# NilanEkanayake/TiTok-Video

Hardware: AMD Instinct MI355X
Metric: video clips/sec encode+decode (whole node) (higher is better)
Workload: dtype bf16

## Files before the change

include/titok_hip.h:

```cpp
#ifndef TITOK_HIP_H
#define TITOK_HIP_H

#include <stdint.h>

#ifdef __cplusplus
extern "C" {
#endif

#define TTV_OK 0
#define TTV_ERR_INVALID 1
#define TTV_ERR_LAUNCH 2
#define TTV_ERR_UNSUPPORTED 3

#define TTV_BF16 0
#define TTV_F32 1

#define TTV_ENCODER 0
#define TTV_DECODER 1

#define TTV_MAX_FSQ 8
#define TTV_MAX_TOKEN 64
#define TTV_MAX_CLIPS_PER_LAUNCH 64

const char* ttv_error_string(void);
// ... 324 lines not shown
  const void* pool_proj_w; const void* pool_proj_b;
  const float* pool_norm2_w; const float* pool_norm2_b;
  const void* pool_fc1_w; const void* pool_fc1_b;
  const void* pool_fc2_w; const void* pool_fc2_b;
} ttv_vjepa_weights;

int ttv_jedi_preprocess(void* const* clips, const int32_t* dims, int n_clips, int dtype, void* out, void* stream);
int64_t ttv_vjepa_workspace_bytes(int n);
int ttv_vjepa_features(const ttv_vjepa_weights* w, const void* x, int n, float* feats, int finetuned, void* workspace,
                       int64_t workspace_bytes, void* stream);

#define TTV_VJEPA_EPI_STORE 0
#define TTV_VJEPA_EPI_GELU 1
#define TTV_VJEPA_EPI_RESID 2
int ttv_vjepa_layernorm(const float* x, int ldx, int rows, int width, const float* w1, const float* b1, float eps1, const float* w2,
                        const float* b2, float eps2, float* y32, int ld32, void* y16, int ld16, void* stream);
int ttv_vjepa_linear(const void* x, int ldx, const void* w, int ldw, const void* bias, int M, int N, int K, int epilogue,
                     const float* resid, int ldr, int resid_rows, void* y, int ldy, void* stream);
int ttv_vjepa_pool_attention(const void* q, const void* kv, int n, int rows, void* out, void* stream);

#define TTV_KC_ATTENTION 1
#define TTV_KC_GEMM_QKV 2
#define TTV_KC_GEMM_GEGLU 3
#define TTV_KC_GEMM_RESID 4
#define TTV_KC_GEMM_STORE 5
#define TTV_KC_RMSNORM 6
#define TTV_KC_PATCH 7
#define TTV_KC_ROWS 8
int ttv_prof_begin(int kernel_class, int max_records);
enum {
  TTV_DBG_NO_STORES = 1,
  TTV_DBG_K256_NO_PANEL_DMA = 2,
  TTV_DBG_MLP_NO_WEIGHT_DMA = 2,
  TTV_DBG_K256_NO_TILE_RELOAD = 4,
  TTV_DBG_MLP_NO_GEGLU = 4,
  TTV_DBG_K256_NO_EPILOGUE_MATH = 8,
  TTV_DBG_MLP_TILES8 = 8,
  TTV_DBG_MLP_NO_P2 = 16,
  TTV_DBG_MLP_PAIRS_ONLY = 32,
  TTV_DBG_MLP_TILES4 = 64,
  TTV_DBG_GEMM_TILE160 = 128,
  TTV_DBG_GEMM_TILE128 = 256,
  TTV_DBG_GEMM_T256 = 512,
  TTV_DBG_MLP_TILES9 = 512,
  TTV_DBG_GEMM_NO_T256 = 1024,
  TTV_DBG_MX_UNFUSED_QUANT = 2048,
  TTV_DBG_SPLIT3_NO_IMAGES = 4096,
  TTV_DBG_SPLIT3_NO_DMA = 8192,
  TTV_DBG_K256_GENERAL = 16384,
  TTV_DBG_QKV256_OFF = 32768,
  TTV_DBG_QKV256_WS = 131072,
  TTV_DBG_ENC_ALL_ROWS = 524288,
  TTV_DBG_ATTN_NO_SWP = 1048576,
  TTV_DBG_DEC_ALL_BLOCKS = 2097152
};
int ttv_debug_set(int flags);
int ttv_debug_stamps(void* device_buffer);
int ttv_prof_end(double* total_ms, int* count);

#ifdef __cplusplus
}
#endif
#endif
```

titok_video_amd/_lib.py:

```python
from __future__ import annotations

import ctypes as C
import os
import threading

import torch

from . import switches

TTV_BF16, TTV_F32 = 0, 1
TTV_ENCODER, TTV_DECODER = 0, 1
TTV_MAX_FSQ = 8
TTV_MAX_TOKEN = 64
TTV_MAX_CLIPS_PER_LAUNCH = 64

DBG_NO_STORES = 1
DBG_K256_NO_PANEL_DMA = 2
DBG_MLP_NO_WEIGHT_DMA = 2
DBG_K256_NO_TILE_RELOAD = 4
DBG_MLP_NO_GEGLU = 4
DBG_K256_NO_EPILOGUE_MATH = 8
DBG_MLP_TILES8 = 8
DBG_MLP_NO_P2 = 16
DBG_MLP_PAIRS_ONLY = 32
DBG_MLP_TILES4 = 64
DBG_GEMM_TILE160 = 128
DBG_GEMM_TILE128 = 256
DBG_GEMM_T256 = 512
DBG_MLP_TILES9 = 512
DBG_GEMM_NO_T256 = 1024
DBG_MX_UNFUSED_QUANT = 2048
DBG_SPLIT3_NO_IMAGES = 4096
DBG_SPLIT3_NO_DMA = 8192
DBG_K256_GENERAL = 16384
DBG_QKV256_OFF = 32768
DBG_QKV256_WS = 131072
DBG_ENC_ALL_ROWS = 524288
DBG_ATTN_NO_SWP = 1048576
DBG_DEC_ALL_BLOCKS = 2097152

_HERE = os.path.dirname(os.path.abspath(__file__))
LIB_PATH = switches.text("TTV_LIB_PATH") or os.path.join(_HERE, "libtitok_hip.so")

i32, i64, f32, vp = C.c_int32, C.c_int64, C.c_float, C.c_void_p


class FsqParams(C.Structure):
    _fields_ = [("n", i32), ("levels", i32 * TTV_MAX_FSQ), ("basis", i32 * TTV_MAX_FSQ),
                ("half_l", f32 * TTV_MAX_FSQ), ("offset", f32 * TTV_MAX_FSQ), ("shift", f32 * TTV_MAX_FSQ),
                ("half_width", f32 * TTV_MAX_FSQ)]


class TowerDims(C.Structure):
    _fields_ = [("kind", i32), ("dtype", i32), ("width", i32), ("layers", i32), ("q_heads", i32), ("kv_heads", i32),
                ("head_dim", i32), ("inner", i32), ("patch_t", i32), ("patch_h", i32), ("patch_w", i32),
                ("pix_channels", i32), ("token_size", i32), ("eps", f32), ("alpha", f32)]


class NextQkv(C.Structure):
    _fields_ = [("qkv", vp), ("ld", i32), ("rope_cs", vp), ("rows", i32), ("rope_q_end", i32), ("rope_k_begin", i32), ("rope_k_end", i32)]


class LayerWeights(C.Structure):
    _fields_ = [("pre_ln", vp), ("to_qkv", vp), ("out_proj", vp), ("ffd_norm", vp), ("w12", vp), ("w3", vp),
                ("attn_post_ln", vp), ("ffd_post_ln", vp), ("to_qkv_pn", vp), ("w12_pn", vp), ("mlp_pack", vp), ("mlp_pack_qkv_rows", i32), ("qkv_q_prescaled", i32),
                ("to_qkv_qs", vp), ("to_qkv_f8", vp), ("to_qkv_f8_scale", vp), ("w12_f8", vp), ("w12_f8_scale", vp),
                ("to_qkv_mx", vp), ("w12_mx", vp), ("out_proj_f8", vp), ("out_proj_f8_scale", vp), ("out_proj_mx", vp),
                ("w3_f8", vp), ("w3_f8_scale", vp), ("w3_mx", vp)]


class TowerWeights(C.Structure):
    _fields_ = [("proj_in_w", vp), ("proj_in_b", vp), ("mask_token", vp), ("ln_pre_t", vp), ("ln_pre_p", vp),
                ("ln_post", vp), ("proj_out_w", vp), ("proj_out_b", vp), ("layers", C.POINTER(LayerWeights)), ("proj_out_pn", vp),
                ("f32_split3", i32)]


class Batch(C.Structure):
    _fields_ = [("n_clips", i32), ("total_rows", i32), ("sum_tokens", i32), ("sum_patches", i32),
                ("max_patches_per_clip", i32), ("n_qblocks", i32), ("cu_seqlens", vp), ("latent_rows", vp),
                ("patch_rows", vp), ("clip_desc", vp), ("qblocks", vp), ("rope_cs", vp), ("blocks64", vp), ("row_seq", vp),
                ("n_blocks64", i32), ("qblocks_paired", i32), ("qblocks_all_full", i32), ("items64", vp), ("n_items64", i32),
                ("rope_ids", vp), ("rope_base", vp), ("qblocks_latent", vp), ("n_qblocks_latent", i32), ("qblocks_patch", vp),
                ("n_qblocks_patch", i32)]


class LayerWeightsT(C.Structure):
    _fields_ = [("to_qkv_t", vp), ("out_proj_t", vp), ("w12_t", vp), ("w3_t", vp)]


class TowerWeightsT(C.Structure):
    _fields_ = [("proj_in_t", vp), ("proj_out_t", vp), ("layers", C.POINTER(LayerWeightsT))]

# ... 200 lines not shown
```

titok_video_amd/csrc/ttv_api.hip:

```cpp
#include <stdarg.h>
#include <stdio.h>
#include <stdlib.h>
#include <string.h>

#include "ttv_common.h"
#include "ttv_kernels.h"

static thread_local char g_err[512] = "";

void ttv_set_error(const char* fmt, ...) {
  va_list ap;
  va_start(ap, fmt);
  vsnprintf(g_err, sizeof(g_err), fmt, ap);
  va_end(ap);
}

int g_ttv_prof_class = 0;
bool ttv_sw_enc_latent_last() { static const bool v = ttv_env_flag("TTV_ENC_LATENT_LAST", true); return v; }
bool ttv_sw_keel_f32sum() { static const bool v = ttv_env_flag("TTV_KEEL_F32SUM", false); return v; }
bool ttv_sw_fused_patch() { static const bool v = ttv_env_flag("TTV_FUSED_PATCH", true); return v; }
bool ttv_sw_attn_pipe() { static const bool v = ttv_env_flag("TTV_ATTN_PIPE", false); return v; }
float ttv_sw_attn_thr() { static const float v = ttv_env_float("TTV_ATTN_THR", 8.0f); return v; }
thread_local int g_ttv_debug = 0;
long long* g_ttv_stamps = nullptr;
static hipEvent_t* g_prof_start = nullptr;
static hipEvent_t* g_prof_stop = nullptr;
static int g_prof_cap = 0, g_prof_n = 0;

TtvProfScope::TtvProfScope(int cls, hipStream_t stream) : slot(-1), s(stream) {
  if (g_ttv_prof_class != 0 && cls == g_ttv_prof_class && g_prof_n < g_prof_cap) {
    slot = g_prof_n++;
    (void)hipEventRecord(g_prof_start[slot], s);
  }
}
TtvProfScope::~TtvProfScope() {
  if (slot >= 0) (void)hipEventRecord(g_prof_stop[slot], s);
}

#define TTV_TRY(expr)            \
  do {                           \
    int rc__ = (expr);           \
    if (rc__ != TTV_OK) return rc__; \
  } while (0)

static inline int esize(int dtype) { return dtype == TTV_BF16 ? 2 : 4; }
static inline int64_t align_up(int64_t v) { return (v + 255) & ~(int64_t)255; }

struct TowerWs {
  char *x, *xn, *qkv, *ao, *h, *pa, *pb;
  char *xl, *aol;
  char *f8, *f8mx;
  float* y32;
  float* rstd;
  int64_t total;
};

static TowerWs carve(const ttv_tower_dims* d, const ttv_batch* b, char* base) {
  const int64_t e = esize(d->dtype);
  const int64_t L = b->total_rows, P = b->sum_patches;
  const int64_t g = (int64_t)d->kv_heads * d->head_dim;
  const int64_t pd = (int64_t)d->pix_channels * d->patch_t * d->patch_h * d->patch_w;
  int64_t off = 0;
  TowerWs w;
  auto take = [&](int64_t bytes) { char* p = base ? base + off : nullptr; off += align_up(bytes); return p; };
  w.x = take(L * d->width * e);
  w.xn = take(L * d->width * e);
  w.qkv = take(L * (2 * d->width + 2 * g) * e);
  w.ao = take(L * d->width * e);
  w.y32 = (float*)take(L * d->width * 4);
  w.h = take(L * d->inner * e);
  w.pa = take(P * pd * e);
  w.pb = take(P * d->width * e);
  w.rstd = (float*)take(L * 4);
// ... 454 lines not shown
  TTV_CHECK_ARG(dtype == TTV_BF16 && head_dim == 64, "attention64: bf16, head_dim 64 only");
  return ttvk_attention64(qkvg, ld, out, ldo, cu_seqlens, items, n_items, q_heads, kv_heads, flags, (hipStream_t)stream);
}

int ttv_patch_gather(const void* const* clips, const int32_t* clip_desc, int clip0, int n_clips, int patch_t, int patch_h, int patch_w,
                     int channels, void* patches, int ld, int dtype, int max_patches_per_clip, void* stream) {
  TTV_CHECK_ARG(n_clips == 0 || (clips && clip_desc && patches), "patch_gather: null buffer");
  return ttvk_patch_copy(false, (void* const*)clips, clip_desc, clip0, n_clips, patch_t, patch_h, patch_w, channels, patches, ld, dtype, max_patches_per_clip, (hipStream_t)stream);
}

int ttv_patch_scatter(const void* patches, int ld, const int32_t* clip_desc, int clip0, int n_clips, int patch_t, int patch_h, int patch_w,
                      int channels, void* const* clips, int dtype, int max_patches_per_clip, void* stream) {
  TTV_CHECK_ARG(n_clips == 0 || (clips && clip_desc && patches), "patch_scatter: null buffer");
  return ttvk_patch_copy(true, clips, clip_desc, clip0, n_clips, patch_t, patch_h, patch_w, channels, (void*)patches, ld, dtype, max_patches_per_clip, (hipStream_t)stream);
}

int64_t ttv_tower_workspace_bytes(const ttv_tower_dims* dims, const ttv_batch* batch) {
  if (check_dims(dims, batch) != TTV_OK) return -1;
  return carve(dims, batch, nullptr).total;
}

int ttv_encoder_forward(const ttv_tower_dims* d, const ttv_tower_weights* w, const ttv_batch* b, const void* const* clips,
                        const ttv_fsq_params* fsq, float* z, void* codes, int32_t* indices, float* bounded, void* workspace,
                        int64_t workspace_bytes, void* stream) {
  TTV_TRY(check_dims(d, b));
  TTV_CHECK_ARG(d->kind == TTV_ENCODER, "encoder_forward: dims.kind is not TTV_ENCODER");
  TTV_CHECK_ARG(w && w->layers && clips && workspace, "encoder_forward: null argument");
  TTV_CHECK_ARG(fsq || z, "encoder_forward: neither fsq nor z requested");
  TTV_CHECK_ARG(!fsq || (codes && indices), "encoder_forward: fsq needs codes and indices buffers");
  hipStream_t s = (hipStream_t)stream;
  TowerWs ws = carve(d, b, (char*)workspace);
  TTV_CHECK_ARG(ws.total <= workspace_bytes, "encoder_forward: workspace too small (%lld < %lld)", (long long)workspace_bytes, (long long)ws.total);
  const int dm = d->width, dt = d->dtype, P = b->sum_patches;
  const int pd = d->pix_channels * d->patch_t * d->patch_h * d->patch_w;

  static const bool use_fused_patch = ttv_sw_fused_patch();
  auto pow2 = [](int v) { return v > 0 && (v & (v - 1)) == 0; };
  const bool gather = use_fused_patch && dt == TTV_BF16 && d->patch_w == 8 && pow2(d->patch_t) && pow2(d->patch_h) &&
                      b->n_clips <= TTV_MAX_CLIPS_PER_LAUNCH && b->row_seq && pd % 64 == 0 && pd != 256;
  if (!gather) {
    for (int c0 = 0; c0 < b->n_clips; c0 += TTV_MAX_CLIPS_PER_LAUNCH) {
      const int n = b->n_clips - c0 < TTV_MAX_CLIPS_PER_LAUNCH ? b->n_clips - c0 : TTV_MAX_CLIPS_PER_LAUNCH;
      TTV_TRY(ttvk_patch_copy(false, (void* const*)(clips + c0), b->clip_desc, c0, n, d->patch_t, d->patch_h, d->patch_w, d->pix_channels, ws.pa, pd, dt, b->max_patches_per_clip, s));
    }
  }
  GemmArgs a = {};
  a.dtype = dt; a.x = ws.pa; a.ldx = pd; a.w = w->proj_in_w; a.ldw = pd; a.M = P; a.N = dm; a.K = pd; a.y = ws.pb; a.ldy = dm;
  a.bias = w->proj_in_b; a.add_scalar = w->mask_token;
  a.split3 = (dt == TTV_F32 && w->f32_split3) ? 1 : 0;
  if (gather) {
    a.gather = 1; a.clips = (void* const*)clips; a.n_clips = b->n_clips; a.clip_desc = b->clip_desc; a.patch_rows = b->patch_rows;
    a.row_seq = b->row_seq; a.patch_t = d->patch_t; a.patch_h = d->patch_h; a.patch_w = d->patch_w;
  }
  TTV_TRY(ttvk_gemm(EPI_STORE, a, s));
  TTV_TRY(ttvk_rmsnorm(ws.pb, dt, dm, nullptr, ws.x, dt, dm, b->patch_rows, w->ln_pre_p, P, dm, d->eps, s));
  TTV_TRY(ttvk_fill_const_rows(ws.x, dt, dm, b->latent_rows, b->sum_tokens, dm, w->mask_token, w->ln_pre_t, d->eps, s));

  TTV_TRY(run_layers(d, w, b, ws, s));

  TTV_TRY(ttvk_enc_tail(ws.x, dt, dm, b->latent_rows, b->sum_tokens, dm, w->ln_post, d->eps, w->proj_out_w, w->proj_out_b, d->token_size, fsq, z, codes, indices, bounded, s));
  return TTV_OK;
}

int ttv_decoder_forward(const ttv_tower_dims* d, const ttv_tower_weights* w, const ttv_batch* b, const void* codes,
                        void* const* clips_out, void* workspace, int64_t workspace_bytes, void* stream) {
  TTV_TRY(check_dims(d, b));
  TTV_CHECK_ARG(d->kind == TTV_DECODER, "decoder_forward: dims.kind is not TTV_DECODER");
  TTV_CHECK_ARG(w && w->layers && codes && clips_out && workspace, "decoder_forward: null argument");
  hipStream_t s = (hipStream_t)stream;
  TowerWs ws = carve(d, b, (char*)workspace);
  TTV_CHECK_ARG(ws.total <= workspace_bytes, "decoder_forward: workspace too small (%lld < %lld)", (long long)workspace_bytes, (long long)ws.total);
  const int dm = d->width, dt = d->dtype, P = b->sum_patches;
  const int pd = d->pix_channels * d->patch_t * d->patch_h * d->patch_w;

  TTV_TRY(ttvk_dec_embed(codes, d->token_size, w->proj_in_w, w->proj_in_b, w->mask_token, w->ln_pre_t, ws.x, dt, dm, b->latent_rows, b->sum_tokens, dm, d->eps, s));
  TTV_TRY(ttvk_fill_const_rows(ws.x, dt, dm, b->patch_rows, P, dm, w->mask_token, w->ln_pre_p, d->eps, s));

  TTV_TRY(run_layers(d, w, b, ws, s));

  GemmArgs a = {};
  a.dtype = dt; a.w = w->proj_out_w; a.ldw = dm; a.M = P; a.N = pd; a.K = dm; a.y = ws.pa; a.ldy = pd; a.ldx = dm;
  a.split3 = (dt == TTV_F32 && w->f32_split3) ? 1 : 0;
  a.bias = w->proj_out_b;
  if (dt == TTV_BF16 && dm == 256 && w->proj_out_pn && pd % 8 == 0) {
    a.x = ws.x; a.x_rows = b->patch_rows; a.w = w->proj_out_pn; a.prenorm = 1; a.eps = d->eps;
  } else {
    TTV_TRY(ttvk_rmsnorm(ws.x, dt, dm, b->patch_rows, ws.pb, dt, dm, nullptr, w->ln_post, P, dm, d->eps, s));
    a.x = ws.pb;
  }
  static const bool use_fused_patch = ttv_sw_fused_patch();
  auto pow2 = [](int v) { return v > 0 && (v & (v - 1)) == 0; };
  if (use_fused_patch && dt == TTV_BF16 && dm == 256 && d->patch_w == 8 && pow2(d->patch_t) && pow2(d->patch_h) &&
      b->n_clips <= TTV_MAX_CLIPS_PER_LAUNCH && b->row_seq && pd % 64 == 0) {
    a.clips = clips_out; a.n_clips = b->n_clips; a.clip_desc = b->clip_desc; a.patch_rows = b->patch_rows; a.row_seq = b->row_seq;
    a.patch_t = d->patch_t; a.patch_h = d->patch_h; a.patch_w = d->patch_w;
    return ttvk_gemm(EPI_STORE_PATCH, a, s);
  }
  TTV_TRY(ttvk_gemm(EPI_STORE, a, s));
  for (int c0 = 0; c0 < b->n_clips; c0 += TTV_MAX_CLIPS_PER_LAUNCH) {
    const int n = b->n_clips - c0 < TTV_MAX_CLIPS_PER_LAUNCH ? b->n_clips - c0 : TTV_MAX_CLIPS_PER_LAUNCH;
    TTV_TRY(ttvk_patch_copy(true, clips_out + c0, b->clip_desc, c0, n, d->patch_t, d->patch_h, d->patch_w, d->pix_channels, ws.pa, pd, dt, b->max_patches_per_clip, s));
  }
  return TTV_OK;
}

int ttv_rope_table_build(const float* base_cos, const float* base_sin, int n_ids, int n_freqs, const int32_t* clip_desc, const int32_t* cu_seqlens,
                         const int32_t* row_seq, float* rope_cs, int total_rows, void* stream) {
  TTV_CHECK_ARG(total_rows == 0 || (base_cos && base_sin && clip_desc && cu_seqlens && row_seq && rope_cs), "rope_table_build: null buffer");
  TTV_CHECK_ARG(n_freqs >= 1 && 3 * n_freqs <= 32 && n_ids >= 1, "rope_table_build: bad table shape");
// ... 183 lines not shown
```

titok_video_amd/csrc/ttv_common.h:

```cpp
#pragma once
#include <hip/hip_runtime.h>
#include <stdint.h>
#include <stdlib.h>

#include "../../include/titok_hip.h"

typedef __bf16 bf16_t;
typedef __attribute__((ext_vector_type(8))) __bf16 bf16x8;
typedef __attribute__((ext_vector_type(4))) __bf16 bf16x4;
typedef __attribute__((ext_vector_type(2))) __bf16 bf16x2;
typedef __attribute__((ext_vector_type(4))) float f32x4;
typedef __attribute__((ext_vector_type(16))) float f32x16;

#define TTV_WAVE 64

void ttv_set_error(const char* fmt, ...);
#define TTV_CHECK_ARG(cond, ...)          \
  do {                                    \
    if (!(cond)) {                        \
      ttv_set_error(__VA_ARGS__);         \
      return TTV_ERR_INVALID;             \
    }                                     \
  } while (0)
#define TTV_CHECK_LAUNCH(what)                                            \
// ... 100 lines not shown
  const unsigned b0 = b[0], b1 = b[1];
  return __uint_as_float(b0) + __uint_as_float(b1);
}
__device__ __forceinline__ float quad16_max(float v) {
  const unsigned u = __float_as_uint(v);
  const auto a = __builtin_amdgcn_permlane16_swap(u, u, false, false);
  const unsigned a0 = a[0], a1 = a[1];
  const float s = fmaxf(__uint_as_float(a0), __uint_as_float(a1));
  const unsigned t = __float_as_uint(s);
  const auto b = __builtin_amdgcn_permlane32_swap(t, t, false, false);
  const unsigned b0 = b[0], b1 = b[1];
  return fmaxf(__uint_as_float(b0), __uint_as_float(b1));
}
__device__ __forceinline__ float pair32_sum(float v) {
  const unsigned u = __float_as_uint(v);
  const auto b = __builtin_amdgcn_permlane32_swap(u, u, false, false);
  const unsigned b0 = b[0], b1 = b[1];
  return __uint_as_float(b0) + __uint_as_float(b1);
}
__device__ __forceinline__ uint4 xchg16_pair(uint2 p0, uint2 p1) {
  const auto x = __builtin_amdgcn_permlane16_swap(p0.x, p1.x, false, false);
  const auto y = __builtin_amdgcn_permlane16_swap(p0.y, p1.y, false, false);
  const unsigned x0 = x[0], x1 = x[1], y0 = y[0], y1 = y[1];
  return make_uint4(x0, y0, x1, y1);
}

extern int g_ttv_prof_class;
extern thread_local int g_ttv_debug;
extern long long* g_ttv_stamps;
struct TtvProfScope {
  int slot;
  hipStream_t s;
  TtvProfScope(int cls, hipStream_t stream);
  ~TtvProfScope();
};

static inline int ttv_cdiv(int a, int b) { return (a + b - 1) / b; }

static inline bool ttv_env_flag(const char* name, bool default_on) {
  const char* v = getenv(name);
  return default_on ? !(v && v[0] == '0') : (v && v[0] == '1');
}
static inline int ttv_env_int(const char* name, int dflt) {
  const char* v = getenv(name);
  return v ? atoi(v) : dflt;
}
static inline float ttv_env_float(const char* name, float dflt) {
  const char* v = getenv(name);
  return v ? (float)atof(v) : dflt;
}
bool ttv_sw_enc_latent_last();
bool ttv_sw_keel_f32sum();
bool ttv_sw_fused_patch();
bool ttv_sw_attn_pipe();
float ttv_sw_attn_thr();

__device__ __forceinline__ float ttv_cubic_src(int dst, float scale) { return fmaf(scale, (float)dst + 0.5f, -0.5f); }
__device__ __forceinline__ int ttv_cubic_floor(int dst, float scale) { return (int)floorf(ttv_cubic_src(dst, scale)); }
__device__ __forceinline__ void cubic_taps(int dst, int n_in, int n_out, int (&idx)[4], float (&w)[4]) {
  const float scale = (float)n_in / (float)n_out;
  const float src = ttv_cubic_src(dst, scale);
  const float fl = floorf(src);
  const float t = src - fl;
  const int i0 = (int)fl;
  constexpr float A = -0.75f;
  auto c1 = [](float x) { return ((A + 2.f) * x - (A + 3.f)) * x * x + 1.f; };
  auto c2 = [](float x) { return ((A * x - 5.f * A) * x + 8.f * A) * x - 4.f * A; };
  w[0] = c2(t + 1.f); w[1] = c1(t); w[2] = c1(1.f - t); w[3] = c2(2.f - t);
#pragma unroll
  for (int k = 0; k < 4; ++k) {
    const int j = i0 - 1 + k;
    idx[k] = j < 0 ? 0 : (j > n_in - 1 ? n_in - 1 : j);
  }
}
typedef float f32x2 __attribute__((ext_vector_type(2)));
__device__ __forceinline__ float geglu_fast(float g, float x) {
  const float gc = __builtin_amdgcn_fmed3f(g, -8.0f, 8.0f);
  const float g2 = gc * gc;
  float q = fmaf(g2, 1.014262858e-03f, -1.067757308e-01f);
  q = fmaf(q, g2, -2.301121361e+00f);
  const float e = __builtin_amdgcn_exp2f(q * gc);
  return (g * __builtin_amdgcn_rcpf(1.0f + e)) * x;
}
__device__ __forceinline__ f32x2 geglu_pair_fast(f32x2 g, f32x2 x) { return (f32x2){geglu_fast(g.x, x.x), geglu_fast(g.y, x.y)}; }

__device__ __forceinline__ void geglu_fast8(const float (&g)[8], const float (&x)[8], float (&h)[8]) {
  float a[8], e[8];
#pragma unroll
  for (int k = 0; k < 8; ++k) {
    const float gc = __builtin_amdgcn_fmed3f(g[k], -8.0f, 8.0f);
    const float g2 = gc * gc;
    float q = fmaf(g2, 1.014262858e-03f, -1.067757308e-01f);
    q = fmaf(q, g2, -2.301121361e+00f);
    a[k] = q * gc;
  }
  __builtin_amdgcn_sched_barrier(0);
#pragma unroll
  for (int k = 0; k < 8; ++k) e[k] = __builtin_amdgcn_exp2f(a[k]);
  __builtin_amdgcn_sched_barrier(0);
#pragma unroll
  for (int k = 0; k < 8; ++k) e[k] = 1.0f + e[k];
  __builtin_amdgcn_sched_barrier(0);
#pragma unroll
  for (int k = 0; k < 8; ++k) e[k] = __builtin_amdgcn_rcpf(e[k]);
  __builtin_amdgcn_sched_barrier(0);
#pragma unroll
// ... 3 lines not shown
```

titok_video_amd/csrc/ttv_gemm.hip:

```cpp
#include <stdlib.h>

#include "ttv_common.h"
#include "ttv_kernels.h"

struct GemmDev {
  const void* x; const void* w; void* y;
  const void* bias; const float* add_scalar; const void* resid; const float* rope_cs;
  int ldx, ldw, ldy, ldr;
  int M, N, K;
  int w_rows;
  float alpha;
  int rope_q_end, rope_k_begin, rope_k_end;
  float eps;
  int debug;
  const float* norm_gain;
  ClipPtrs clips;
  const int* clip_desc; const int* patch_rows; const int* row_seq;
  const int* x_rows;
  const float* row_scale;
  const int* rope_ids; const float* rope_base;
  const float* x_scale; const float* w_scale;
  float* sum_f32; int ld_sum;
  void* y2; int ldy2; const float* norm_gain2;
  int split3;
// ... 1175 lines not shown
    }
    __builtin_amdgcn_s_waitcnt(0x0F70);
    __syncthreads();
    if (it + 1 < it1) {
      LOADA(af[0], buf ^ 1, 0);
      if (K256_DEPTH == 3) LOADA(af[1], buf ^ 1, 1);
    }

    int tok[2];
#pragma unroll
    for (int j = 0; j < 2; ++j) {
      tok[j] = tile * K256_TT + wave * 32 + j * 16 + l15;
      if (PRENORM && !(p.debug & TTV_DBG_K256_NO_EPILOGUE_MATH)) {
#pragma unroll
        for (int i = 0; i < 4; ++i) acc[i][j] *= rstd[j];
      }
    }
    if (DUAL) {
      int feat[2] = {panel * FO + kq * 4, panel * FO + 16 + kq * 4};
      f32x4 ax[2][2] = {{acc[0][0], acc[0][1]}, {acc[1][0], acc[1][1]}};
      f32x4 ag[2][2] = {{acc[2][0], acc[2][1]}, {acc[3][0], acc[3][1]}};
      epilogue_tile<EPI, bf16_t, 2, 2>(p, tok, feat, ax, ag, kq);
    } else if (EPI == EPI_QKV_ROPE) {
      int feat[4];
#pragma unroll
      for (int i = 0; i < 4; ++i) feat[i] = panel * FO + i * 16 + kq * 4;
      const int f_first = panel * FO;
      if (!(p.debug & TTV_DBG_K256_NO_EPILOGUE_MATH) && (f_first < p.rope_q_end || (f_first >= p.rope_k_begin && f_first < p.rope_k_end))) {
#pragma unroll
        for (int i = 0; i < 4; ++i)
#pragma unroll
          for (int j = 0; j < 2; ++j) {
            const f32x4 a = acc[i][j];
            acc[i][j] = (f32x4){a[0] * rc[i][j].x - a[1] * rs[i][j].x, a[0] * rs[i][j].x + a[1] * rc[i][j].x,
                                a[2] * rc[i][j].y - a[3] * rs[i][j].y, a[2] * rs[i][j].y + a[3] * rc[i][j].y};
          }
      }
      epilogue_tile<EPI_STORE, bf16_t, 4, 2>(p, tok, feat, acc, acc, kq);
    } else {
      int feat[4];
#pragma unroll
      for (int i = 0; i < 4; ++i) feat[i] = panel * FO + i * 16 + kq * 4;
      epilogue_tile<EPI, bf16_t, 4, 2>(p, tok, feat, acc, acc, kq, EPI == EPI_STORE_PATCH ? pdst : nullptr);
    }
  }
#undef WROWIDX
#undef GLDS_PANEL
#undef LOADA
#undef MFMA8
}

#include "ttv_qkv256.inc"
#include "ttv_qkv256ws.inc"

#define ROW_TT 64

__global__ __launch_bounds__(256, 2) void k_gemm_k256_rownorm(GemmDev p, int n_tiles) {
  __shared__ uint4 wl[2][K256_ROWS * 32];
  const int tid = threadIdx.x, lane = tid & 63, wave = tid >> 6;
  const int l15 = lane & 15, kq = lane >> 4;
  if ((int)blockIdx.x >= n_tiles) return;
  const bf16_t* W = (const bf16_t*)p.w;
  const bf16_t* X = (const bf16_t*)p.x;
  const int srow = tid >> 5, sch = tid & 31;
  uint4 st0, st1, st2, st3, st4, st5, st6, st7;
#define WROWN(panel_, i_) (*reinterpret_cast<const uint4*>(W + (size_t)((panel_) * 64 + srow + 8 * (i_)) * p.ldw + sch * 8))
#define GLOADN(panel_)                                                                                       \
  do {                                                                                                       \
    st0 = WROWN(panel_, 0); st1 = WROWN(panel_, 1); st2 = WROWN(panel_, 2); st3 = WROWN(panel_, 3);          \
    st4 = WROWN(panel_, 4); st5 = WROWN(panel_, 5); st6 = WROWN(panel_, 6); st7 = WROWN(panel_, 7);          \
  } while (0)
#define LIDXN(i_) ((srow + 8 * (i_)) * 32 + ((sch & 16) | ((sch & 15) ^ ((srow + 8 * (i_)) & 15))))
#define LSTOREN(buf_)                                                                                        \
  do {                                                                                                       \
    wl[buf_][LIDXN(0)] = st0; wl[buf_][LIDXN(1)] = st1; wl[buf_][LIDXN(2)] = st2; wl[buf_][LIDXN(3)] = st3;  \
    wl[buf_][LIDXN(4)] = st4; wl[buf_][LIDXN(5)] = st5; wl[buf_][LIDXN(6)] = st6; wl[buf_][LIDXN(7)] = st7;  \
  } while (0)

  GLOADN(0);
  LSTOREN(0);
  __syncthreads();
  for (int tile = blockIdx.x; tile < n_tiles; tile += gridDim.x) {
    const bool last_tile = tile + (int)gridDim.x >= n_tiles;
    int t = tile * ROW_TT + wave * 16 + l15;
    const bool tvalid = t < p.M;
    t = tvalid ? t : p.M - 1;
    bf16x8 bfr[8];
    {
      const bf16_t* xr = X + (size_t)t * p.ldx + kq * 8;
#pragma unroll
      for (int s8 = 0; s8 < 8; ++s8) bfr[s8] = *reinterpret_cast<const bf16x8*>(xr + s8 * 32);
    }
    f32x4 acc[16];
#pragma unroll
    for (int i = 0; i < 16; ++i) acc[i] = (f32x4){0.f, 0.f, 0.f, 0.f};
#pragma unroll
    for (int panel = 0; panel < 4; ++panel) {
      const int buf = panel & 1;
      const bool more = !(last_tile && panel == 3);
      if (more) GLOADN((panel + 1) & 3);
#pragma unroll
      for (int s8 = 0; s8 < 8; ++s8) {
        const int ch = s8 * 4 + kq;
        bf16x8 a[4];
#pragma unroll
        for (int i = 0; i < 4; ++i) {
// ... 798 lines not shown
```

titok_video_amd/csrc/ttv_kernels.h:

```cpp
#pragma once
#include <hip/hip_runtime.h>
#include <stdint.h>

#include "../../include/titok_hip.h"

int ttvk_rmsnorm(const void* in, int in_dtype, int ld_in, const int* src_rows, void* out, int out_dtype, int ld_out,
                 const int* dst_rows, const float* gain, int rows, int d, float eps, hipStream_t s, float* next_rstd = nullptr,
                 void* mx_q = nullptr, void* mx_s = nullptr,
                 int split_image = 0);
int ttvk_row_rstd(const void* in, int dtype, int ld_in, float* rstd, int rows, int d, float eps, hipStream_t s);
int ttvk_copy_rows(const void* src, int64_t ld_src_bytes, const int* src_rows, void* dst, int64_t ld_dst_bytes, const int* dst_rows, int rows,
                   int row_bytes, hipStream_t s);
int ttvk_fill_const_rows(void* x, int dtype, int ld, const int* rows_map, int rows, int d, const float* mask_token,
                         const float* gain, float eps, hipStream_t s);
int ttvk_dec_embed(const void* codes, int C, const void* w, const void* bias, const float* mask_token, const float* gain,
                   void* x, int dtype, int ld, const int* rows_map, int rows, int d, float eps, hipStream_t s);
int ttvk_fsq_forward(const ttv_fsq_params* p, const void* z, int z_dtype, int rows, void* codes, int codes_dtype, int* indices,
                     float* bounded, hipStream_t s);
int ttvk_fsq_indices_to_codes(const ttv_fsq_params* p, const int* indices, int rows, void* codes, int codes_dtype, hipStream_t s);
int ttvk_enc_tail(const void* x, int dtype, int ld, const int* rows_map, int rows, int d, const float* gain, float eps,
                  const void* w, const void* bias, int C, const ttv_fsq_params* fsq, float* z_out, void* codes, int* indices,
                  float* bounded, hipStream_t s);
int ttvk_patch_copy(bool scatter, void* const* clips, const int* clip_desc, int clip0, int n_clips, int pt, int ph, int pw,
                    int C, void* patches, int ld, int dtype, int max_patches, hipStream_t s);
// ... 7 lines not shown
int ttvk_quant_mx_fp8(const void* in, int in_dtype, int ld_in, void* out, int ld_out, void* mx, float* row_scales, int rows, int d, hipStream_t s);

int ttvk_clip_from_u8(const void* frames, long long n_pix, void* clip, int dtype, hipStream_t s);

int ttvk_clip_resample_u8(void* const* src, void* const* dst, const int32_t* geom, int n_clips, int dtype, hipStream_t s);

enum GemmEpilogue {
  EPI_STORE = 0,
  EPI_QKV_ROPE,
  EPI_GEGLU,
  EPI_RESID_T,
  EPI_RESID_F32,
  EPI_RESID_NORM,
  EPI_STORE_PATCH,
  EPI_BIAS_PLAIN,
  EPI_BIAS_GELU,
  EPI_BIAS_RESID_F32R,
};

struct GemmArgs {
  const void* x; int ldx;
  const void* w; int ldw;
  int M, N, K;
  void* y; int ldy;
  const void* bias;
  const float* add_scalar;
  const void* resid; int ldr;
  float alpha;
  const float* rope_cs;
  const int* rope_ids; const float* rope_base;
  int rope_q_end, rope_k_begin, rope_k_end;
  int dtype;
  const float* norm_gain;
  float* sum_f32; int ld_sum;
  void* y2; int ldy2; const float* norm_gain2;
  void* yq; void* yq_mx;
  int split3;
  int x_image, y_image;
  int prenorm;
  const float* row_scale;
  const int* x_rows;
  float eps;
  int gather;
  void* const* clips;
  int n_clips;
  const int* clip_desc;
  const int* patch_rows;
  const int* row_seq;
  int patch_t, patch_h, patch_w;
  int resid_rows;
};
struct ClipPtrs { void* p[TTV_MAX_CLIPS_PER_LAUNCH]; };
int ttvk_gemm(GemmEpilogue epi, const GemmArgs& a, hipStream_t s);
int ttvk_gemm_fp8(GemmEpilogue epi, const GemmArgs& a, const float* x_scale, const float* w_scale, hipStream_t s, const void* x_mx = nullptr,
                  const void* w_mx = nullptr);
bool ttvk_gemm_supports_resid_norm(int dtype, int N, int K);

int ttvk_attention(const void* qkvg, int ld, void* out, int ldo, const int* cu_seqlens, const int* qblocks, int n_qblocks,
                   int q_heads, int kv_heads, int head_dim, int flags, int dtype, hipStream_t s, float* lse_out = nullptr,
                   void* out_raw = nullptr);

int ttvk_attention_swp(const void* qkvg, int ld, void* out, int ldo, const int* cu_seqlens, const int* qblocks, int n_qblocks,
                       int q_heads, int kv_heads, int gate_mul, hipStream_t s);
int ttvk_attention_mxout(const void* qkvg, int ld, void* out_q, void* out_mx, int ld_mx, const int* cu_seqlens, const int* qblocks,
                         int n_qblocks, int q_heads, int kv_heads, hipStream_t s);

int ttvk_attention64(const void* qkvg, int ld, void* out, int ldo, const int* cu_seqlens, const int* items, int n_items, int q_heads,
                     int kv_heads, int flags, hipStream_t s);

int ttvk_vq_norms(const void* cb, int dtype, int ld, int N, int C, float* cnorm, hipStream_t s);
int64_t ttvk_vq_workspace_bytes(int rows);
int ttvk_vq_l2_argmin(const void* z, int dtype, int ldz, const void* cb, int ldc, const float* cnorm, int rows, int N, int C, int* indices,
                      float* best_dist, void* workspace, int64_t workspace_bytes, hipStream_t s);
int ttvk_vq_lookup(const void* cb, int dtype, int ldc, const int* indices, int rows, int C, void* codes, int ldo, hipStream_t s);
int ttvk_vq_lookup_bwd(const void* dcodes, int dtype, int ld, const int* indices, int rows, int C, float* dcb, int ldc, hipStream_t s);

bool ttvk_mlp_fused_supported(int dtype, int width, int inner);
struct MlpNextQkv {
  void* qkv; int ld;
  const float* rope_cs;
  int rows;
  int rope_q_end, rope_k_begin, rope_k_end;
};
int64_t ttvk_mlp_pack_bytes(int inner, int next_qkv_rows);
int ttvk_mlp_pack(const void* w12_folded, const void* w3, const void* wo, const void* next_qkv_folded, int next_qkv_rows, int inner,
                  void* packed, hipStream_t s);
int ttvk_mlp_fused(const void* ao, int ldao, const float* front_gain, float front_alpha, const void* x, int ldx, const void* packed,
                   int inner, void* y, int ldy, const float* post_gain, float alpha, float eps, int M, const MlpNextQkv* nq, hipStream_t s);

int ttvk_l1_loss(void* const* recon, void* const* target, void* const* grad, const int* sizes, int n_clips, int total_clips, int dtype,
                 float* loss, hipStream_t s);
int ttvk_sq_err(void* const* recon, void* const* target, const int* sizes, int n_clips, int dtype, int clamp, double* acc2, hipStream_t s);
int ttvk_rmsnorm_bwd_chain(const void* x, int ldx, const void* dy, int lddy, const float* gain1, float* dgain1, float* dx, int lddx,
                           const void* y, int y_dt, int ldy, const float* gain2, float* dgain2, float out_scale, void* cast_out, int ldc, int rows,
                           int d, float eps, int dt, hipStream_t s);
int ttvk_rmsnorm_bwd(const void* x, int x_dt, int ldx, const int* xr, const void* dy, int dy_dt, int lddy, const int* dyr,
                     const float* gain, void* dx, int dx_dt, int lddx, const int* dxr, int acc, float* dgain, int rows, int d, float eps,
                     hipStream_t s);
int ttvk_colsum(const void* a, int dt, int lda, const int* rows_map, int rows, int n, float* out, hipStream_t s);
int ttvk_sumall(const void* a, int dt, int lda, const int* rows_map, int rows, int n, const float* colw, float scale, float* out, hipStream_t s);
int ttvk_gate_fwd(const void* a, int lda, const void* gate, int ldg, void* ag, int ldo, int rows, int d, int dt, hipStream_t s);
int ttvk_gate_bwd(const void* dag, int ldd, const void* a, int lda, const void* gate, int ldg, void* da, int ldda, void* dgate, int lddg,
                  int rows, int d, int dt, float* delta, hipStream_t s);
int ttvk_geglu_fwd(const void* u, int ldu, void* h, int ldh, int rows, int I, int dt, hipStream_t s);
int ttvk_geglu_bwd(const void* u, int ldu, const void* dh, int lddh, void* du, int lddu, int rows, int I, int dt, hipStream_t s);
int ttvk_scale_cast(const float* a, float alpha, float* b, void* c, int dt, long n, hipStream_t s);
// ... 68 lines not shown
```

Before: 30170.

## Fuse encoder patch-gather GEMM, pre-norm RMSNorm and latent mask fill into one kernel

Adds a dedicated encoder input kernel that gathers patches straight from the clips into LDS via async global-to-LDS loads, runs the projection GEMM with MFMA using a triple-buffered pipeline, then applies bias, mask scalar, RMSNorm and the pre-norm gain in the epilogue before writing rows to the token buffer. The same kernel also fills the constant latent rows. This replaces three launches and the intermediate round trip through the patch buffer. It is specialised to width 256 and bf16, and it uses inline asm that touches m0.

```diff
diff --git a/include/titok_hip.h b/include/titok_hip.h
--- a/include/titok_hip.h
+++ b/include/titok_hip.h
@@ -400,7 +400,8 @@
   TTV_DBG_QKV256_WS = 131072,
   TTV_DBG_ENC_ALL_ROWS = 524288,
   TTV_DBG_ATTN_NO_SWP = 1048576,
-  TTV_DBG_DEC_ALL_BLOCKS = 2097152
+  TTV_DBG_DEC_ALL_BLOCKS = 2097152,
+  TTV_DBG_NO_PATCH_EMBED = 4194304
 };
 int ttv_debug_set(int flags);
 int ttv_debug_stamps(void* device_buffer);
diff --git a/titok_video_amd/_lib.py b/titok_video_amd/_lib.py
--- a/titok_video_amd/_lib.py
+++ b/titok_video_amd/_lib.py
@@ -38,6 +38,7 @@
 DBG_ENC_ALL_ROWS = 524288
 DBG_ATTN_NO_SWP = 1048576
 DBG_DEC_ALL_BLOCKS = 2097152
+DBG_NO_PATCH_EMBED = 4194304
 
 _HERE = os.path.dirname(os.path.abspath(__file__))
 LIB_PATH = switches.text("TTV_LIB_PATH") or os.path.join(_HERE, "libtitok_hip.so")
diff --git a/titok_video_amd/csrc/ttv_api.hip b/titok_video_amd/csrc/ttv_api.hip
--- a/titok_video_amd/csrc/ttv_api.hip
+++ b/titok_video_amd/csrc/ttv_api.hip
@@ -19,6 +19,7 @@
 bool ttv_sw_enc_latent_last() { static const bool v = ttv_env_flag("TTV_ENC_LATENT_LAST", true); return v; }
 bool ttv_sw_keel_f32sum() { static const bool v = ttv_env_flag("TTV_KEEL_F32SUM", false); return v; }
 bool ttv_sw_fused_patch() { static const bool v = ttv_env_flag("TTV_FUSED_PATCH", true); return v; }
+bool ttv_sw_patch_embed() { static const bool v = ttv_env_flag("TTV_PATCH_EMBED", true); return v; }
 bool ttv_sw_attn_pipe() { static const bool v = ttv_env_flag("TTV_ATTN_PIPE", false); return v; }
 float ttv_sw_attn_thr() { static const float v = ttv_env_float("TTV_ATTN_THR", 8.0f); return v; }
 thread_local int g_ttv_debug = 0;
@@ -579,9 +580,16 @@
     a.gather = 1; a.clips = (void* const*)clips; a.n_clips = b->n_clips; a.clip_desc = b->clip_desc; a.patch_rows = b->patch_rows;
     a.row_seq = b->row_seq; a.patch_t = d->patch_t; a.patch_h = d->patch_h; a.patch_w = d->patch_w;
   }
-  TTV_TRY(ttvk_gemm(EPI_STORE, a, s));
-  TTV_TRY(ttvk_rmsnorm(ws.pb, dt, dm, nullptr, ws.x, dt, dm, b->patch_rows, w->ln_pre_p, P, dm, d->eps, s));
-  TTV_TRY(ttvk_fill_const_rows(ws.x, dt, dm, b->latent_rows, b->sum_tokens, dm, w->mask_token, w->ln_pre_t, d->eps, s));
+  static const bool use_patch_embed = ttv_sw_patch_embed();
+  GemmArgs pe = a;
+  pe.y = ws.x; pe.norm_gain = w->ln_pre_p; pe.eps = d->eps;
+  if (gather && use_patch_embed && !(g_ttv_debug & TTV_DBG_NO_PATCH_EMBED) && ttvk_patch_embed_supported(pe)) {
+    TTV_TRY(ttvk_patch_embed(pe, b->latent_rows, b->sum_tokens, w->ln_pre_t, s));
+  } else {
+    TTV_TRY(ttvk_gemm(EPI_STORE, a, s));
+    TTV_TRY(ttvk_rmsnorm(ws.pb, dt, dm, nullptr, ws.x, dt, dm, b->patch_rows, w->ln_pre_p, P, dm, d->eps, s));
+    TTV_TRY(ttvk_fill_const_rows(ws.x, dt, dm, b->latent_rows, b->sum_tokens, dm, w->mask_token, w->ln_pre_t, d->eps, s));
+  }
 
   TTV_TRY(run_layers(d, w, b, ws, s));
 
diff --git a/titok_video_amd/csrc/ttv_common.h b/titok_video_amd/csrc/ttv_common.h
--- a/titok_video_amd/csrc/ttv_common.h
+++ b/titok_video_amd/csrc/ttv_common.h
@@ -176,6 +176,7 @@
 bool ttv_sw_enc_latent_last();
 bool ttv_sw_keel_f32sum();
 bool ttv_sw_fused_patch();
+bool ttv_sw_patch_embed();
 bool ttv_sw_attn_pipe();
 float ttv_sw_attn_thr();
 
diff --git a/titok_video_amd/csrc/ttv_gemm.hip b/titok_video_amd/csrc/ttv_gemm.hip
--- a/titok_video_amd/csrc/ttv_gemm.hip
+++ b/titok_video_amd/csrc/ttv_gemm.hip
@@ -1251,6 +1251,7 @@
 
 #include "ttv_qkv256.inc"
 #include "ttv_qkv256ws.inc"
+#include "ttv_patch_embed.inc"
 
 #define ROW_TT 64
 
diff --git a/titok_video_amd/csrc/ttv_kernels.h b/titok_video_amd/csrc/ttv_kernels.h
--- a/titok_video_amd/csrc/ttv_kernels.h
+++ b/titok_video_amd/csrc/ttv_kernels.h
@@ -83,6 +83,8 @@
 };
 struct ClipPtrs { void* p[TTV_MAX_CLIPS_PER_LAUNCH]; };
 int ttvk_gemm(GemmEpilogue epi, const GemmArgs& a, hipStream_t s);
+bool ttvk_patch_embed_supported(const GemmArgs& a);
+int ttvk_patch_embed(const GemmArgs& a, const int* latent_rows, int n_latent, const float* latent_gain, hipStream_t s);
 int ttvk_gemm_fp8(GemmEpilogue epi, const GemmArgs& a, const float* x_scale, const float* w_scale, hipStream_t s, const void* x_mx = nullptr,
                   const void* w_mx = nullptr);
 bool ttvk_gemm_supports_resid_norm(int dtype, int N, int K);
diff --git a/titok_video_amd/csrc/ttv_patch_embed.inc b/titok_video_amd/csrc/ttv_patch_embed.inc
--- /dev/null
+++ b/titok_video_amd/csrc/ttv_patch_embed.inc
@@ -0,0 +1,198 @@
+#define PE_TT 128
+#define PE_STAGE ((256 + PE_TT) * 8)
+#define PE_PITCH 528
+
+__global__ __launch_bounds__(512) void k_patch_embed(GemmDev p, const int* __restrict__ latent_rows, int n_latent,
+                                                     const float* __restrict__ latent_gain) {
+  __shared__ __attribute__((aligned(16))) uint4 lds[3 * PE_STAGE];
+  const int tid = threadIdx.x, lane = tid & 63;
+  const int wave = __builtin_amdgcn_readfirstlane(tid >> 6);
+  const int wf = wave & 3, wt = wave >> 2;
+  const int tbase = blockIdx.x * PE_TT;
+  const bf16_t* W = (const bf16_t*)p.w;
+
+  const int lr = lane >> 3, lp = lane & 7;
+  uint32_t woff[4];
+#pragma unroll
+  for (int i = 0; i < 4; ++i) {
+    const int row = wave * 32 + i * 8 + lr;
+    woff[i] = ((uint32_t)row * (uint32_t)p.ldw + (uint32_t)((lp ^ ((row >> 1) & 7)) * 8)) * 2u;
+  }
+  const bf16_t* xb[2];
+  int xthw[2], xhw[2], xw[2], xch[2];
+#pragma unroll
+  for (int i = 0; i < 2; ++i) {
+    const int row = wave * 16 + i * 8 + lr;
+    int t = tbase + row;
+    t = t < p.M ? t : p.M - 1;
+    const int ci = p.row_seq[p.patch_rows[t]];
+    const int* ds = p.clip_desc + (size_t)ci * 8;
+    const int Tn = ds[0], H = ds[1], Wd = ds[2], gh = ds[4], gw = ds[5], pl = t - ds[6];
+    const int gwi = pl % gw, r = pl / gw, ghi = r % gh, gti = r / gh;
+    xthw[i] = Tn * H * Wd; xhw[i] = H * Wd; xw[i] = Wd;
+    xch[i] = lp ^ ((row >> 1) & 7);
+    xb[i] = reinterpret_cast<const bf16_t*>(p.clips.p[ci - p.clip0]) + ((size_t)((gti << p.pt_shift) * H + (ghi << p.ph_shift)) * Wd + gwi * 8);
+  }
+  const uint32_t lds0 = (uint32_t)(uintptr_t)(__attribute__((address_space(3))) void*)&lds[0];
+  constexpr uint32_t STAGEB = PE_STAGE * 16;
+#define PE_STAGE_LOAD(kt_, buf_)                                                                                 \
+  do {                                                                                                           \
+    const bf16_t* wb__ = W + (size_t)(kt_) * BK;                                                                 \
+    const uint32_t dw__ = lds0 + (buf_) * STAGEB + wave * 4096;                                                  \
+    const uint32_t dx__ = lds0 + (buf_) * STAGEB + 256 * 128 + wave * 2048;                                      \
+    _Pragma("unroll") for (int i__ = 0; i__ < 4; ++i__) {                                                        \
+      unsigned keep__;                                                                                           \
+      asm volatile("s_mov_b32 %0, m0\n\ts_mov_b32 m0, %3\n\ts_nop 0\n\tglobal_load_lds_dwordx4 %1, %2\n\ts_mov_b32 m0, %0" \
+                   : "=&s"(keep__) : "v"(woff[i__]), "s"(wb__), "s"(dw__ + i__ * 1024) : "memory");               \
+    }                                                                                                            \
+    _Pragma("unroll") for (int i__ = 0; i__ < 2; ++i__) {                                                        \
+      const int sg__ = (kt_) * 8 + xch[i__];                                                                     \
+      const int c__ = sg__ >> (p.pt_shift + p.ph_shift), ipt__ = (sg__ >> p.ph_shift) & ((1 << p.pt_shift) - 1); \
+      const int iph__ = sg__ & ((1 << p.ph_shift) - 1);                                                          \
+      const bf16_t* src__ = xb[i__] + ((size_t)c__ * xthw[i__] + (size_t)ipt__ * xhw[i__] + (size_t)iph__ * xw[i__]); \
+      unsigned keep__;                                                                                           \
+      asm volatile("s_mov_b32 %0, m0\n\ts_mov_b32 m0, %2\n\ts_nop 0\n\tglobal_load_lds_dwordx4 %1, off\n\ts_mov_b32 m0, %0" \
+                   : "=&s"(keep__) : "v"(src__), "s"(dx__ + i__ * 1024) : "memory");                              \
+    }                                                                                                            \
+  } while (0)
+#define PE_FENCE() __builtin_amdgcn_sched_barrier(0)
+
+  f32x4 acc[4][4];
+#pragma unroll
+  for (int i = 0; i < 4; ++i)
+#pragma unroll
+    for (int j = 0; j < 4; ++j) acc[i][j] = (f32x4){0.f, 0.f, 0.f, 0.f};
+
+  const int l15 = lane & 15, kq = lane >> 4;
+  const int nk = p.K / BK;
+  PE_FENCE();
+  asm volatile("s_waitcnt vmcnt(0)" ::: "memory");
+  PE_FENCE();
+  PE_STAGE_LOAD(0, 0);
+  if (nk > 1) PE_STAGE_LOAD(1, 1);
+  int buf = 0;
+  for (int kt = 0; kt < nk; ++kt) {
+    PE_FENCE();
+    if (kt + 1 < nk) asm volatile("s_waitcnt vmcnt(6)\n\ts_barrier" ::: "memory");
+    else asm volatile("s_waitcnt vmcnt(0)\n\ts_barrier" ::: "memory");
+    PE_FENCE();
+    if (kt + 2 < nk) {
+      const int nb = buf == 0 ? 2 : buf - 1;
+      PE_STAGE_LOAD(kt + 2, nb);
+    }
+    const uint4* sw = lds + buf * PE_STAGE;
+    const uint4* sx = sw + 256 * 8;
+#pragma unroll
+    for (int ks = 0; ks < 2; ++ks) {
+      bf16x8 a[4], b[4];
+      const int kc = ks * 4 + kq;
+#pragma unroll
+      for (int i = 0; i < 4; ++i) {
+        const int arow = wf * 64 + i * 16 + l15;
+        a[i] = __builtin_bit_cast(bf16x8, sw[arow * 8 + (kc ^ ((arow >> 1) & 7))]);
+      }
+#pragma unroll
+      for (int j = 0; j < 4; ++j) {
+        const int brow = wt * 64 + j * 16 + l15;
+        b[j] = __builtin_bit_cast(bf16x8, sx[brow * 8 + (kc ^ ((brow >> 1) & 7))]);
+      }
+#pragma unroll
+      for (int i = 0; i < 4; ++i)
+#pragma unroll
+        for (int j = 0; j < 4; ++j) acc[i][j] = __builtin_amdgcn_mfma_f32_16x16x32_bf16(a[i], b[j], acc[i][j], 0, 0, 0);
+    }
+    buf = buf == 2 ? 0 : buf + 1;
+  }
+#undef PE_STAGE_LOAD
+
+  char* const tile = reinterpret_cast<char*>(lds);
+  {
+    const float sc = round_to<bf16_t>(p.add_scalar[0]);
+    f32x4 bias[4];
+#pragma unroll
+    for (int i = 0; i < 4; ++i) bias[i] = Vec4<bf16_t>::load((const bf16_t*)p.bias + wf * 64 + i * 16 + kq * 4);
+    __syncthreads();
+#pragma unroll
+    for (int i = 0; i < 4; ++i)
+#pragma unroll
+      for (int j = 0; j < 4; ++j) {
+        acc[i][j] += bias[i];
+#pragma unroll
+        for (int e = 0; e < 4; ++e) acc[i][j][e] = round_to<bf16_t>(acc[i][j][e]);
+        acc[i][j] += sc;
+        const int row = wt * 64 + j * 16 + l15, feat = wf * 64 + i * 16 + kq * 4;
+        *reinterpret_cast<uint2*>(tile + row * PE_PITCH + feat * 2) = pack_bf16x4(acc[i][j]);
+      }
+    __syncthreads();
+  }
+
+  {
+    const int c = lane * 4;
+    const f32x4 g = *reinterpret_cast<const f32x4*>(p.norm_gain + c);
+    const float eps = p.eps;
+    bf16_t* const out = (bf16_t*)p.y;
+    const int t_l = tbase + wave * 16 + l15;
+    const int dst_l = p.patch_rows[t_l < p.M ? t_l : p.M - 1];
+#pragma unroll
+    for (int r0 = 0; r0 < 16; r0 += 4) {
+      f32x4 v[4];
+      float ss[4];
+#pragma unroll
+      for (int q = 0; q < 4; ++q) {
+        v[q] = Vec4<bf16_t>::load(reinterpret_cast<const bf16_t*>(tile + (wave * 16 + r0 + q) * PE_PITCH) + c);
+        ss[q] = 0.f;
+        ss[q] += v[q][0] * v[q][0] + v[q][1] * v[q][1] + v[q][2] * v[q][2] + v[q][3] * v[q][3];
+      }
+#pragma unroll
+      for (int q = 0; q < 4; ++q) ss[q] = wave_sum(ss[q]);
+#pragma unroll
+      for (int q = 0; q < 4; ++q) {
+        const float rstd = 1.0f / sqrtf(ss[q] / 256.0f + eps);
+        const f32x4 o = {v[q][0] * rstd * g[0], v[q][1] * rstd * g[1], v[q][2] * rstd * g[2], v[q][3] * rstd * g[3]};
+        const int dst = __builtin_amdgcn_readlane(dst_l, r0 + q);
+        if (tbase + wave * 16 + r0 + q < p.M) Vec4<bf16_t>::store(out + (size_t)dst * p.ldy + c, o);
+      }
+    }
+  }
+
+  {
+    const int c = lane * 4;
+    const float m = round_to<bf16_t>(p.add_scalar[0]);
+    const float rstd = 1.0f / sqrtf(m * m + p.eps);
+    const f32x4 g = *reinterpret_cast<const f32x4*>(latent_gain + c);
+    const f32x4 o = {m * rstd * g[0], m * rstd * g[1], m * rstd * g[2], m * rstd * g[3]};
+    bf16_t* const out = (bf16_t*)p.y;
+    for (int r = blockIdx.x * 8 + wave; r < n_latent; r += gridDim.x * 8) Vec4<bf16_t>::store(out + (size_t)latent_rows[r] * p.ldy + c, o);
+  }
+#undef PE_FENCE
+}
+
+bool ttvk_patch_embed_supported(const GemmArgs& a) {
+  auto pow2 = [](int v) { return v > 0 && (v & (v - 1)) == 0; };
+  return a.dtype == TTV_BF16 && a.N == 256 && a.K > 0 && a.K % BK == 0 && a.ldw == a.K && a.ldy % 4 == 0 && a.patch_w == 8 && pow2(a.patch_t) &&
+         pow2(a.patch_h) && a.n_clips > 0 && a.n_clips <= TTV_MAX_CLIPS_PER_LAUNCH && a.bias && a.add_scalar && a.norm_gain &&
+         (uint64_t)a.N * (uint64_t)a.ldw * 2u < (1ull << 32);
+}
+
+int ttvk_patch_embed(const GemmArgs& a, const int* latent_rows, int n_latent, const float* latent_gain, hipStream_t s) {
+  if (a.M == 0) return ttvk_fill_const_rows(a.y, a.dtype, a.ldy, latent_rows, n_latent, a.N, a.add_scalar, latent_gain, a.eps, s);
+  if (!ttvk_patch_embed_supported(a)) {
+    ttv_set_error("patch_embed: needs bf16, width 256, K %% 64 == 0, patch_w == 8, power-of-two patch_t / patch_h, bias and mask_token");
+    return TTV_ERR_UNSUPPORTED;
+  }
+  TTV_CHECK_ARG(a.clips && a.clip_desc && a.patch_rows && a.row_seq && a.w && a.y && (n_latent == 0 || (latent_rows && latent_gain)),
+                "patch_embed: null buffer");
+  TTV_CHECK_ARG(((uintptr_t)a.w % 16 == 0) && ((uintptr_t)a.y % 8 == 0) && ((uintptr_t)a.norm_gain % 16 == 0) && ((uintptr_t)a.bias % 8 == 0) &&
+                (n_latent == 0 || (uintptr_t)latent_gain % 16 == 0), "patch_embed: unaligned buffer");
+  auto lg2 = [](int v) { int sh = 0; while ((1 << sh) < v) ++sh; return sh; };
+  GemmDev d = {};
+  d.w = a.w; d.y = a.y; d.bias = a.bias; d.add_scalar = a.add_scalar; d.ldw = a.ldw; d.ldy = a.ldy; d.M = a.M; d.N = a.N; d.K = a.K; d.w_rows = a.N;
+  d.eps = a.eps; d.norm_gain = a.norm_gain; d.debug = g_ttv_debug;
+  d.clip_desc = a.clip_desc; d.patch_rows = a.patch_rows; d.row_seq = a.row_seq; d.clip0 = 0;
+  for (int i = 0; i < a.n_clips; ++i) d.clips.p[i] = a.clips[i];
+  d.pt_shift = lg2(a.patch_t); d.ph_shift = lg2(a.patch_h);
+  TtvProfScope prof(TTV_KC_GEMM_STORE, s);
+  hipLaunchKernelGGL(k_patch_embed, dim3(ttv_cdiv(a.M, PE_TT)), dim3(512), 0, s, d, latent_rows, n_latent, latent_gain);
+  TTV_CHECK_LAUNCH("patch_embed");
+  return TTV_OK;
+}
```

Measured after the change: 30520 (median of 6 runs). About the same (+1.2%).
